# YukinoriMatsuoka/indy-plenum

Hardware: AMD Instinct MI355X
Metric: Ed25519 verifies/sec at 1/8 MI355X (256B msgs) + % of INT32 VALU peak vs host CPU (higher is better)
Workload: dtype int32

## Files before the change

indy-plenum_amd/csrc/edv_hostcheck.cpp:

```cpp
#include <stdint.h>
#include <string.h>
#include <vector>
#include "edv_verify_core.h"
#include "edv_sha256.h"
#include "edv_merkle.h"
#include "edv_ledger.h"
#include "edv_tables.h"
#include "edv_selftest_cases.h"
#include "edv_probe_ops.h"

using namespace edv;

namespace {
struct HostATab {
  ge_cached t[kAEntries];
  int staged = 0;
  void store(int e, const ge_cached& c) { t[e] = c; }
  ge_cached load(int e) const { return t[e]; }
  void stage(int e) { staged = e; }
  ge_cached fetch() const { return t[staged]; }
};
struct HostBTab {
  SbShape sh;
  ge_p3 base[kBTablesCompact];
  explicit HostBTab(SbShape s) : sh(s) {
    for (int t = 0; t < sh.tables; t++) base[t] = base_point(t * sh.bits);
  }
  ge_precomp entry(int t, int j) const {
    int32_t w[kBStride];
    btab_entry(w, j, base[t]);
    return precomp_from_words(w);
  }
};
struct HostBStage {
  const HostBTab& b;
  int t = 0, j = 0;
  ge_cached stash;
  SbShape shape() const { return b.sh; }
  void stage(int tt, int jj) { t = tt; j = jj; }
  ge_precomp fetch() const { return b.entry(t, j); }
  void put(const ge_cached& c) { stash = c; }
  ge_cached get() const { return stash; }
};
struct HostComb {
  std::vector<int32_t> w;
  HostComb() : w(kCombRows * kCombEntries * kBStride) {
    for (int i = 0; i < kCombRows; i++)
      for (int j = 0; j < kCombEntries; j++) comb_entry(w.data() + (i * kCombEntries + j) * kBStride, i, j);
  }
  ge_precomp entry(int i, int j) const { return precomp_from_words(w.data() + (i * kCombEntries + j) * kBStride); }
};
const HostComb& comb() {
  static HostComb c;
  return c;
}
static_assert(kBTablesCompact >= kBTables, "base[] holds the larger table count");
const HostBTab& btab(int bits = kBBits) {
  static HostBTab large(sb_large()), compact(sb_compact());
  return bits == kBBitsCompact ? compact : large;
}
void load_words(uint32_t* w, const uint8_t* b, int n) {
  for (int i = 0; i < n; i++) w[i] = uint32_t(b[4 * i]) | uint32_t(b[4 * i + 1]) << 8 | uint32_t(b[4 * i + 2]) << 16 | uint32_t(b[4 * i + 3]) << 24;
}
void store_words(uint8_t* b, const uint32_t* w, int n) {
  for (int i = 0; i < n; i++)
    for (int j = 0; j < 4; j++) b[4 * i + j] = uint8_t(w[i] >> (8 * j));
}
fe to_fe(const int32_t* l) { fe f; for (int i = 0; i < 10; i++) f.v[i] = l[i]; return f; }
void from_fe(int32_t* l, const fe& f) { for (int i = 0; i < 10; i++) l[i] = f.v[i]; }
}

extern "C" {
void hc_fe_mul(const int32_t* f, const int32_t* g, int32_t* h) { from_fe(h, fe_mul(to_fe(f), to_fe(g))); }
void hc_fe_sq(const int32_t* f, int32_t* h) { from_fe(h, fe_sq(to_fe(f))); }
void hc_fe_sq_floor(const int32_t* f, int32_t* h) { from_fe(h, fe_sq_floor(to_fe(f))); }
void hc_fe_sq2(const int32_t* f, int32_t* h) { from_fe(h, fe_sq2(to_fe(f))); }
void hc_fe_carry32(const int32_t* f, int32_t* h) { from_fe(h, fe_carry32(to_fe(f))); }
void hc_fe_invert(const int32_t* f, int32_t* h) { from_fe(h, fe_invert(to_fe(f))); }
void hc_fe_invert_safegcd(const int32_t* f, int32_t* h) { from_fe(h, fe_invert_safegcd(to_fe(f))); }
void hc_fe_pow22523(const int32_t* f, int32_t* h) { from_fe(h, fe_pow22523(to_fe(f))); }
void hc_fe_tobytes(const int32_t* f, uint8_t* out) { uint32_t w[8]; fe_tobytes(w, to_fe(f)); store_words(out, w, 8); }
void hc_fe_frombytes(const uint8_t* in, int32_t* h) { uint32_t w[8]; load_words(w, in, 8); from_fe(h, fe_frombytes(w)); }
void hc_sc_reduce(const uint8_t* in64, uint8_t* out32) {
  uint32_t w[16], o[8];
  load_words(w, in64, 16);
  sc_reduce(o, w);
  store_words(out32, o, 8);
}
void hc_hram(const uint8_t* R, const uint8_t* A, const uint8_t* m, uint64_t mlen, uint8_t* out64) {
  uint32_t r[8], a[8], o[16];
  load_words(r, R, 8);
  load_words(a, A, 8);
  std::vector<uint8_t> buf(mlen + 32, 0);
  if (mlen) memcpy(buf.data() + 16, m, mlen);
  hram(o, r, a, buf.data() + 16, mlen);
  store_words(out64, o, 16);
}
int hc_decompress_negate(const uint8_t* in, uint8_t* out) {
  uint32_t w[8], o[8];
  load_words(w, in, 8);
  ge_p3 p;
  const bool ok = ge_frombytes_negate(p, w);
  ge_p2_tobytes(o, ge_p3_to_p2(p));
  store_words(out, o, 8);
  return ok ? 0 : -1;
}
void hc_sha256(const uint8_t* m, uint64_t mlen, int misalign, uint8_t* out32) {
  std::vector<uint8_t> buf(mlen + 48, 0xA5);
  if (mlen) memcpy(buf.data() + 16 + misalign, m, mlen);
  uint32_t o[8];
  sha256_msg(o, buf.data() + 16 + misalign, mlen);
  store_words(out32, o, 8);
}
int hc_sha256_batch(const uint8_t* msgs, const uint64_t* off, uint64_t n, uint8_t* out, uint32_t) {
  for (uint64_t i = 0; i < n; i++) {
    const uint64_t mlen = off[i + 1] - off[i];
    std::vector<uint8_t> buf(mlen + 48, 0);
    if (mlen) memcpy(buf.data() + 16, msgs + off[i], mlen);
    uint32_t o[8];
    sha256_msg(o, buf.data() + 16, mlen);
    store_words(out + 32 * i, o, 8);
  }
  return 0;
}
int hc_btab_entries_of_bits(int bits, int t, const int32_t* js, int nj, int32_t* out) {
  if (bits != kBBits && bits != kBBitsCompact) return -1;
  const HostBTab& b = btab(bits);
  if (t < 0 || t >= b.sh.tables) return -1;
  for (int k = 0; k < nj; k++) {
    if (js[k] < 0 || js[k] >= b.sh.entries) return -1;
    btab_entry(out + size_t(k) * kBStride, js[k], b.base[t]);
  }
  return 0;
}
int hc_btab_entries_of(int t, const int32_t* js, int nj, int32_t* out) {
  return hc_btab_entries_of_bits(kBBits, t, js, nj, out);
}
int hc_rside_point_bits(int bits, const uint8_t* R32, const uint8_t* S32, uint8_t* out32) {
  struct Keep {
    ge_cached q;
    void store(int e, const ge_cached& c) { if (e == 1) q = c; }
  } tab;
  uint32_t R[8], S[8], o[8];
  load_words(R, R32, 8);
  load_words(S, S32, 8);
  if (bits != kBBits && bits != kBBitsCompact) return -1;
  HostBStage bs{btab(bits)};
  if (!prep_rpoint(R, S, tab, bs)) return -1;
  const fe two_y = fe_carry32(fe_add(tab.q.YpX, tab.q.YmX)), two_x = fe_carry32(fe_sub(tab.q.YpX, tab.q.YmX));
  ge_p2 p{two_x, two_y, fe_carry32(fe_add(tab.q.Z, tab.q.Z))};
  ge_p2_tobytes(o, p);
  store_words(out32, o, 8);
  return 0;
}
int hc_rside_point(const uint8_t* R32, const uint8_t* S32, uint8_t* out32) {
  return hc_rside_point_bits(kBBits, R32, S32, out32);
}
int hc_half_scalars(const uint8_t* h32, uint8_t* a32, uint8_t* u32) {
  uint32_t h[8], a[8], u[8];
  load_words(h, h32, 8);
  bool neg = false;
  half_scalars(h, a, u, neg);
  store_words(a32, a, 8);
  store_words(u32, u, 8);
  return neg ? 1 : 0;
}
int hc_probe_math(int op, const void* in, uint64_t in_stride, void* out, uint64_t out_stride, uint64_t n) {
  const ProbeSize sz = probe_size(op);
  if (!sz.in || probe_is_quad(op) || in_stride < sz.in || out_stride < sz.out || (in_stride & 3) || (out_stride & 3))
    return -1;
  for (uint64_t i = 0; i < n; i++) {
    const uint32_t* x = reinterpret_cast<const uint32_t*>(static_cast<const uint8_t*>(in) + i * in_stride);
    uint32_t* y = reinterpret_cast<uint32_t*>(static_cast<uint8_t*>(out) + i * out_stride);
    switch (op) {
#define HC_PROBE_CASE(OP) case OP: probe_lane_op<OP>(x, y); break;
      HC_PROBE_CASE(EDV_PROBE_FE_MUL)
      HC_PROBE_CASE(EDV_PROBE_FE_SQ)
      HC_PROBE_CASE(EDV_PROBE_FE_SQ2)
      HC_PROBE_CASE(EDV_PROBE_FE_SQ_FLOOR)
      HC_PROBE_CASE(EDV_PROBE_FE_TOBYTES)
      HC_PROBE_CASE(EDV_PROBE_FE_FROMBYTES)
      HC_PROBE_CASE(EDV_PROBE_FE_INVERT_SAFEGCD)
      HC_PROBE_CASE(EDV_PROBE_FE_POW22523)
      HC_PROBE_CASE(EDV_PROBE_SC_REDUCE)
      HC_PROBE_CASE(EDV_PROBE_HALF_SCALARS)
      HC_PROBE_CASE(EDV_PROBE_RECODE5)
      HC_PROBE_CASE(EDV_PROBE_APPROX_DIV)
      HC_PROBE_CASE(EDV_PROBE_FDIV_FLOOR)
      HC_PROBE_CASE(EDV_PROBE_EUCLID_DIV)
      HC_PROBE_CASE(EDV_PROBE_GE_FROMBYTES)
      HC_PROBE_CASE(EDV_PROBE_SC_MULADD)
      HC_PROBE_CASE(EDV_PROBE_RECODE8)
      HC_PROBE_CASE(EDV_PROBE_GE_P3_TOBYTES)
#undef HC_PROBE_CASE
      case EDV_PROBE_SCALARMULT_BASE: probe_scalarmult_base(x, y, comb()); break;
      default: return -1;
    }
  }
  return 0;
}
static_assert(kAEntries * 40 == 360, "a slot's table is 9 entries of 4 x 10 limbs");
int hc_stage_prep(const uint8_t* sigs, const uint8_t* pks, const uint8_t* msgs, const uint64_t* off, uint64_t n,
                  int bits, int side0, int nsides, int buckets, uint64_t cap, uint32_t* dig, uint8_t* alive,
                  int32_t* atab, int32_t* rtab, uint32_t* perm, uint8_t* accept) {
  if ((bits != kBBits && bits != kBBitsCompact) || n > cap || side0 < 0 || nsides < 1 || side0 + nsides > 3) return -1;
  const HostBTab& bt = btab(bits);
  if (buckets) {
    auto bucket = [&](uint64_t i) {
      const uint64_t nb = (64 + (off[i + 1] - off[i]) + 17 + 127) / 128;
      return nb < 63 ? nb : uint64_t(63);
    };
    uint64_t k = 0;
    bool one = true;
    for (uint64_t i = 1; i < n; i++) one = one && bucket(i) == bucket(0);
    for (uint64_t b = 0; b < 64 && !one; b++)
      for (uint64_t i = 0; i < n; i++)
        if (bucket(i) == b) perm[k++] = uint32_t(i);
    for (uint64_t i = 0; one && i < n; i++) perm[i] = uint32_t(i);
  }
  for (uint64_t j = 0; j < n; j++) {
    const uint64_t i = buckets ? perm[j] : j;
    uint32_t R[8], S[8], A[8];
    load_words(R, sigs + 64 * i, 8);
    load_words(S, sigs + 64 * i + 32, 8);
    load_words(A, pks + 32 * i, 8);
    for (int side = side0; side < side0 + nsides; side++) {
      bool ok;
      if (side == 0) {
        const uint64_t mlen = off[i + 1] - off[i];
        std::vector<uint8_t> buf(mlen + 32, 0);
        if (mlen) memcpy(buf.data() + 16, msgs + off[i], mlen);
        PrepDigits pd;
        ok = prep_one(R, S, A, buf.data() + 16, mlen, pd);
        if (ok) {
          for (int k = 0; k < 8; k++) {
            dig[uint64_t(k) * cap + j] = pd.da[k];
            dig[uint64_t(8 + k) * cap + j] = pd.db[k];
          }
          dig[16 * cap + j] = uint32_t(pd.nwin) | (pd.negR ? 0x100u : 0u);
        }
      } else {
        HostATab tab;
        if (side == 1) {
          ok = prep_point(A, tab);
        } else {
          HostBStage bs{bt};
          ok = prep_rpoint(R, S, tab, bs);
        }
        int32_t* o = (side == 1 ? atab : rtab) + j * 360;
        for (int e = 0; ok && e < kAEntries; e++) {
          from_fe(o + 40 * e, tab.t[e].YpX);
          from_fe(o + 40 * e + 10, tab.t[e].YmX);
          from_fe(o + 40 * e + 20, tab.t[e].Z);
          from_fe(o + 40 * e + 30, tab.t[e].T2d);
        }
      }
      alive[uint64_t(side) * cap + j] = ok ? 1 : 0;
      if (!ok) accept[i] = 0;
    }
  }
  return 0;
}
int hc_stage_main(uint64_t n, uint64_t cap, const uint32_t* dig, const uint8_t* alive, const int32_t* atab,
                  const int32_t* rtab, const uint32_t* perm, uint8_t* accept) {
  if (n > cap) return -1;
  auto live = [&](uint64_t j) { return j < n && alive[j] && alive[cap + j] && alive[2 * cap + j]; };
  for (uint64_t w0 = 0; w0 < n; w0 += 64) {
    int nwin = 0;
    for (uint64_t j = w0; j < w0 + 64; j++)
      if (live(j)) nwin = mx(nwin, int(dig[16 * cap + j] & 0xff));
    if (nwin > kAWindows) return -1;
    for (uint64_t j = w0; j < w0 + 64; j++) {
      if (!live(j)) continue;
      if (perm && perm[j] >= n) return -1;
      uint32_t da[8], db[8];
      for (int k = 0; k < 8; k++) {
        da[k] = dig[uint64_t(k) * cap + j];
        db[k] = dig[uint64_t(8 + k) * cap + j];
      }
      HostATab at, rt;
      for (int e = 0; e < kAEntries; e++) {
        const int32_t *a = atab + j * 360 + 40 * e, *r = rtab + j * 360 + 40 * e;
        at.t[e] = ge_cached{to_fe(a), to_fe(a + 10), to_fe(a + 20), to_fe(a + 30)};
        rt.t[e] = ge_cached{to_fe(r), to_fe(r + 10), to_fe(r + 20), to_fe(r + 30)};
      }
      accept[perm ? perm[j] : j] = main_one(da, db, nwin, (dig[16 * cap + j] >> 8) & 1, at, rt) ? 1 : 0;
    }
  }
  return 0;
}
namespace {
void put_p3(int32_t* pt, int k, uint64_t slots, uint64_t j, const ge_p3& p) {
  const fe* c[4] = {&p.X, &p.Y, &p.Z, &p.T};
  for (int q = 0; q < 4; q++)
    for (int i = 0; i < 10; i++) pt[(uint64_t(k) * 40 + 10 * q + i) * slots + j] = c[q]->v[i];
}
ge_p3 get_p3(const int32_t* pt, int k, uint64_t slots, uint64_t j) {
  fe c[4];
  for (int q = 0; q < 4; q++)
    for (int i = 0; i < 10; i++) c[q].v[i] = pt[(uint64_t(k) * 40 + 10 * q + i) * slots + j];
  return ge_p3{c[0], c[1], c[2], c[3]};
}
ge_p3 p3_add(const ge_p3& p, const ge_p3& q) { return ge_p1p1_to_p3(ge_add(p, ge_p3_to_cached(q))); }
ge_p3 p3_neg(const ge_p3& p) { return ge_p3{fe_neg(p.X), p.Y, p.Z, fe_neg(p.T)}; }
ge_p3 signed_digit_mult(const uint32_t d[8], bool negate, const ge_p3& P) {
  ge_p3 m[9];
  m[0] = ge_p3_identity();
  for (int e = 1; e < 9; e++) m[e] = p3_add(m[e - 1], P);
  ge_p3 acc = ge_p3_identity();
  for (int k = 63; k >= 0; k--) {
    for (int t = 0; t < 4; t++) acc = ge_p1p1_to_p3(ge_p2_dbl(ge_p3_to_p2(acc)));
    int dg = int(d[k / 8] >> (4 * (k % 8))) & 15;
    if (dg >= 8) dg -= 16;
    if (negate) dg = -dg;
    if (dg) acc = p3_add(acc, dg < 0 ? p3_neg(m[-dg]) : m[dg]);
  }
  return acc;
}
}
int hc_stage_latency_phase1(const uint8_t* sigs, const uint8_t* pks, const uint8_t* msgs, const uint64_t* off,
                            uint64_t n, int ns, int bits, uint32_t* dig, int32_t* pt, uint8_t* ok) {
  if ((bits != kBBits && bits != kBBitsCompact) || (ns != 16 && ns != 32) || n == 0) return -1;
  const HostBTab& bt = btab(bits);
  const uint64_t slots = (n + ns - 1) / ns * ns;
  for (uint64_t jl = 0; jl < slots; jl++) {
    const bool in = jl < n || jl < 16;
    const uint64_t i = jl < n ? jl : n - 1;
    bool ok0 = false, ok1 = false, ok2 = false;
    PrepDigits pd;
    ge_p3 pa = ge_p3_identity(), pr = ge_p3_identity(), sb = ge_p3_identity();
    if (in) {
      uint32_t R[8], S[8], A[8];
      load_words(R, sigs + 64 * i, 8);
      load_words(S, sigs + 64 * i + 32, 8);
      load_words(A, pks + 32 * i, 8);
      const uint64_t mlen = off[i + 1] - off[i];
      std::vector<uint8_t> buf(mlen + 32, 0);
      if (mlen) memcpy(buf.data() + 16, msgs + off[i], mlen);
      ok0 = prep_one(R, S, A, buf.data() + 16, mlen, pd);
      ok1 = ge_is_canonical(A) && !has_small_order(A) && ge_frombytes_negate(pa, A);
      if (!ok1) pa = ge_p3_identity();
      ok2 = ge_is_canonical(R) && !has_small_order(R) && ge_frombytes_negate(pr, R);
      if (!ok2) pr = ge_p3_identity();
      HostBStage bs{bt};
      add_sb(sb, S, bs);
    }
    for (int k = 0; k < 8; k++) {
      dig[uint64_t(k) * slots + jl] = ok0 ? pd.da[k] : 0u;
      dig[uint64_t(8 + k) * slots + jl] = ok0 ? pd.db[k] : 0u;
    }
    dig[16 * slots + jl] = ok0 ? (uint32_t(pd.nwin) | (pd.negR ? 0x100u : 0u)) : 0u;
    ok[jl] = ok0;
    ok[slots + jl] = ok1;
    ok[2 * slots + jl] = ok2;
    put_p3(pt, 0, slots, jl, pa);
    put_p3(pt, 1, slots, jl, pr);
    put_p3(pt, 2, slots, jl, sb);
  }
  return 0;
}
int hc_stage_latency_walk(uint64_t n, int ns, const uint32_t* dig, const int32_t* pt, const uint8_t* ok,
                          uint8_t* accept) {
  if ((ns != 16 && ns != 32) || n == 0) return -1;
  const uint64_t slots = (n + ns - 1) / ns * ns;
  for (uint64_t j = 0; j < n; j++) {
    const bool alive = ok[j] && ok[slots + j] && ok[2 * slots + j];
    if (!alive) {
      accept[j] = 0;
      continue;
    }
    const uint32_t wf = dig[16 * slots + j];
    if ((wf & 0xff) > uint32_t(kAWindows)) return -1;
    uint32_t da[8], db[8];
    for (int k = 0; k < 8; k++) {
      da[k] = dig[uint64_t(k) * slots + j];
      db[k] = dig[uint64_t(8 + k) * slots + j];
    }
    const ge_p3 q = p3_add(get_p3(pt, 2, slots, j), get_p3(pt, 1, slots, j));
    const ge_p3 r = p3_add(signed_digit_mult(da, false, get_p3(pt, 0, slots, j)),
                           signed_digit_mult(db, (wf >> 8) & 1, q));
    accept[j] = (fe_iszero(r.X) && fe_iszero(fe_sub(r.Y, r.Z))) ? 1 : 0;
  }
  return 0;
}
int hc_comb_entries(const int32_t* ij, int n, int32_t* out) {
  const HostComb& ct = comb();
// ... 185 lines not shown
```

indy-plenum_amd/csrc/edv_prep.hip:

```cpp
#define EDV_NO_SCHED_FENCE 1
#include <hip/hip_runtime.h>
#include <stdint.h>

#include "edv_kernels.h"

namespace edv {
namespace {



template <int BITS>
__device__ __forceinline__ void prep_point_side(const VerifyArgs& a, uint64_t j, int side, int32_t* lds) {
  if (j >= a.n) return;
  const uint64_t i = a.base + (a.st.perm ? a.st.perm[j] : j);
  uint32_t P[8];
  bool ok;
  if (side == 1) {
    load_words(P, a.pks + 8 * i, 2);
    GlobalATab tab{a.st.atab + j * kAWords};
    ok = prep_point(P, tab);
  } else {
    uint32_t S[8];
    load_words(P, a.sigs + 16 * i, 2);
    load_words(S, a.sigs + 16 * i + 8, 2);
    GlobalATab tab{a.st.rtab + j * kAWords};
    LdsBStage<BITS> bs{a.btab, lds + (threadIdx.x >> 6) * kLdsBWaveWords, int(threadIdx.x & 63)};
    ok = prep_rpoint(P, S, tab, bs);
  }
  a.st.alive[side * a.st.cap + j] = ok ? 1 : 0;
  if (!ok) a.accept[i] = 0;
}
template <int BITS>
__device__ __forceinline__ void prep_body(const VerifyArgs& a, int32_t* lds_b) {
  const uint32_t ns = uint32_t(a.nsides);
  const int side = a.side0 + int(blockIdx.x % ns);
  const uint64_t j = uint64_t(blockIdx.x / ns) * kBlock + threadIdx.x;
  if (side != 0) {
    prep_point_side<BITS>(a, j, side, lds_b);
    return;
  }
  if (j >= a.n) return;
  const uint64_t i = a.base + (a.st.perm ? a.st.perm[j] : j);
  uint32_t R[8], S[8], A[8];
  load_words(R, a.sigs + 16 * i, 2);
  load_words(S, a.sigs + 16 * i + 8, 2);
  load_words(A, a.pks + 8 * i, 2);
  const uint64_t o0 = a.off[i] - a.msg_base, o1 = a.off[i + 1] - a.msg_base;
  PrepDigits pd;
  const bool ok = prep_one(R, S, A, a.msgs + o0, o1 - o0, pd);
  a.st.alive[j] = ok ? 1 : 0;
  if (ok) {
    uint32_t* d = a.st.dig + j;
    const uint64_t cap = a.st.cap;
#pragma unroll
    for (int k = 0; k < 8; k++) {
      d[uint64_t(k) * cap] = pd.da[k];
      d[uint64_t(8 + k) * cap] = pd.db[k];
    }
    d[uint64_t(kDigNwin) * cap] = uint32_t(pd.nwin) | (pd.negR ? 0x100u : 0u);
  } else {
    a.accept[i] = 0;
  }
}

__global__ __launch_bounds__(kBlock) __attribute__((amdgpu_waves_per_eu(3, 8))) void edv_prep_kernel(
    VerifyArgs a) {
  extern __shared__ int32_t lds_b[];
  prep_body<kBBits>(a, lds_b);
}
__global__ __launch_bounds__(kBlock) __attribute__((amdgpu_waves_per_eu(3, 8))) void edv_prep_kernel_compact(
    VerifyArgs a) {
  extern __shared__ int32_t lds_b[];
  prep_body<kBBitsCompact>(a, lds_b);
}

}

hipError_t launch_prep_kernel(unsigned grid, hipStream_t s, const VerifyArgs& va) {
  const bool rside = va.side0 + va.nsides > 2;
  const size_t lds = rside ? size_t(kBlock / 64) * kLdsBWaveWords * sizeof(int32_t) : 0;
  if (va.sb.bits == kBBits) edv_prep_kernel<<<dim3(grid), dim3(kBlock), lds, s>>>(va);
  else edv_prep_kernel_compact<<<dim3(grid), dim3(kBlock), lds, s>>>(va);
  return hipGetLastError();
}

}
```

indy-plenum_amd/csrc/edv_verify_core.h:

```cpp
#pragma once
#include "edv_math.h"

namespace edv {

constexpr int kAWin = 4;
constexpr int kAWindows = (255 + kAWin - 1) / kAWin;
constexpr int kAEntries = (1 << (kAWin - 1)) + 1;
constexpr int kBBits = 22;
constexpr int kBTables = (253 + kBBits - 1) / kBBits;
constexpr int kBEntries = (1 << (kBBits - 1)) + 1;
constexpr int kBBitsCompact = 16;
constexpr int kBTablesCompact = (253 + kBBitsCompact - 1) / kBBitsCompact;
constexpr int kBEntriesCompact = (1 << (kBBitsCompact - 1)) + 1;
static_assert(253 - kBBits * (kBTables - 1) <= kBBits - 1, "top [S]B digit out of table range");
static_assert(253 - kBBitsCompact * (kBTablesCompact - 1) <= kBBitsCompact - 1, "top [S]B digit out of table range");
struct SbShape {
  int bits, tables, entries;
};
EDV_HD constexpr SbShape sb_large() { return SbShape{kBBits, kBTables, kBEntries}; }
EDV_HD constexpr SbShape sb_compact() { return SbShape{kBBitsCompact, kBTablesCompact, kBEntriesCompact}; }
constexpr int kCombEntries = 129;
constexpr int kBStride = 32;

EDV_HD int mx(int a, int b) { return a > b ? a : b; }
// ... 146 lines not shown
  for (int k = 0; k < kAWindows; k++) {
    const int pos = kAWin * k, wi = pos >> 5, sh = pos & 31;
    const uint64_t win = uint64_t(d[wi]) | (wi + 1 < 8 ? uint64_t(d[wi + 1]) << 32 : 0);
    n = ((win >> sh) & ((1u << kAWin) - 1)) ? k + 1 : n;
  }
  return n;
}

EDV_HD bool w8_lt(const uint32_t a[8], const uint32_t b[8]) {
  bool lt = false, eq = true;
#pragma unroll
  for (int i = 7; i >= 0; i--) {
    lt = lt || (eq && a[i] < b[i]);
    eq = eq && a[i] == b[i];
  }
  return lt;
}
EDV_HD void w8_add(uint32_t a[8], const uint32_t b[8]) {
  uint64_t c = 0;
#pragma unroll
  for (int i = 0; i < 8; i++) {
    c += uint64_t(a[i]) + b[i];
    a[i] = uint32_t(c);
    c >>= 32;
  }
}
EDV_HD void w8_sub(uint32_t a[8], const uint32_t b[8]) {
  int64_t br = 0;
#pragma unroll
  for (int i = 0; i < 8; i++) {
    const int64_t s = int64_t(a[i]) - int64_t(b[i]) + br;
    a[i] = uint32_t(s);
    br = s >> 32;
  }
}
EDV_HD double w8_to_f64(const uint32_t a[8]) {
  double d = 0.0;
#pragma unroll
  for (int i = 7; i >= 0; i--) d = d * 4294967296.0 + double(a[i]);
  return d;
}
EDV_HD void w8_shl1(uint32_t a[8]) {
#pragma unroll
  for (int i = 7; i > 0; i--) a[i] = (a[i] << 1) | (a[i - 1] >> 31);
  a[0] <<= 1;
}
EDV_HD void w8_sar1(uint32_t a[8]) {
#pragma unroll
  for (int i = 0; i < 7; i++) a[i] = (a[i] >> 1) | (a[i + 1] << 31);
  a[7] = uint32_t(int32_t(a[7]) >> 1);
}
EDV_HD void w8_shr1(uint32_t a[8]) {
#pragma unroll
  for (int i = 0; i < 7; i++) a[i] = (a[i] >> 1) | (a[i + 1] << 31);
  a[7] >>= 1;
}

#ifndef EDV_RCP_DIV
#define EDV_RCP_DIV 1
#endif
EDV_HD double approx_div(double a, double b) {
#if defined(__HIP_DEVICE_COMPILE__)
  if (EDV_RCP_DIV) {
    double r = __builtin_amdgcn_rcp(b);
    r = __builtin_fma(r, __builtin_fma(-b, r, 1.0), r);
    return a * r;
  }
#endif
  return a / b;
}
EDV_HD void euclid_div(uint32_t r0[8], uint32_t t0[8], const uint32_t r1[8], const uint32_t t1[8]) {
  const double qd = __builtin_floor(approx_div(w8_to_f64(r0), w8_to_f64(r1)) * (1.0 - 0x1p-44));
  uint32_t q = 0;
  if (qd < 2147483648.0) {
    q = uint32_t(qd);
    uint64_t c = 0;
    int64_t br = 0;
#pragma unroll
    for (int i = 0; i < 8; i++) {
      const uint64_t p = uint64_t(q) * r1[i] + c;
      c = p >> 32;
      const int64_t s = int64_t(r0[i]) - int64_t(uint32_t(p)) + br;
      r0[i] = uint32_t(s);
      br = s >> 32;
    }
  } else {
    uint32_t d[8], v[8];
#pragma unroll
    for (int i = 0; i < 8; i++) { d[i] = r1[i]; v[i] = t1[i]; }
    const int e = int((__builtin_bit_cast(uint64_t, qd * (1.0 + 0x1p-42)) >> 52) & 0x7ff) - 1023;
#pragma unroll 1
    for (int k = 0; k < e; k++) { w8_shl1(d); w8_shl1(v); }
#pragma unroll 1
    for (int k = e; k >= 0; k--) {
      if (!w8_lt(r0, d)) { w8_sub(r0, d); w8_sub(t0, v); }
      w8_shr1(d);
      w8_sar1(v);
    }
  }
  const uint32_t m = w8_lt(r0, r1) ? 0u : ~0u;
  int64_t br = 0;
#pragma unroll
  for (int i = 0; i < 8; i++) {
    const int64_t s = int64_t(r0[i]) - int64_t(r1[i] & m) + br;
    r0[i] = uint32_t(s);
    br = s >> 32;
  }
  q -= m;
  uint64_t c = 0;
  int64_t bt = 0;
#pragma unroll
  for (int i = 0; i < 8; i++) {
    const uint64_t p = uint64_t(q) * t1[i] + c;
    c = p >> 32;
    const int64_t s = int64_t(t0[i]) - int64_t(uint32_t(p)) + bt;
    t0[i] = uint32_t(s);
    bt = s >> 32;
  }
}

EDV_HD bool w8_ge128(const uint32_t r[8]) { return (r[4] | r[5] | r[6] | r[7]) != 0; }

EDV_HD double w8_window53(const uint32_t r[8], int s) {
  const int wi = s >> 5, b = s & 31;
  uint32_t w0 = 0, w1 = 0, w2 = 0;
#pragma unroll
  for (int k = 0; k < 8; k++) {
    const uint32_t d = uint32_t(k - wi);
    const uint32_t m0 = ~nz_mask(d), m1 = ~nz_mask(d - 1u), m2 = ~nz_mask(d - 2u);
    w0 |= r[k] & m0;
    w1 |= r[k] & m1;
    w2 |= r[k] & m2;
  }
  const uint64_t lo = (uint64_t(w1) << 32) | w0;
  const uint64_t v = b == 0 ? lo : ((lo >> b) | (uint64_t(w2) << (64 - b)));
  return double(v);
}
EDV_HD double fdiv_floor(double a, double b) {
  double q = __builtin_floor(approx_div(a, b));
  const double r = __builtin_fma(-q, b, a);
  q = r < 0 ? q - 1 : (r >= b ? q + 1 : q);
  return q;
}
EDV_HD void w8_lin(uint32_t out[8], const uint32_t x[8], const uint32_t y[8], int32_t a, int32_t b) {
  int64_t c = 0;
#pragma unroll
  for (int i = 0; i < 8; i++) {
    const int64_t v = int64_t(a) * int64_t(uint64_t(x[i])) + int64_t(b) * int64_t(uint64_t(y[i])) + c;
    out[i] = uint32_t(v);
    c = v >> 32;
  }
}

EDV_HD bool lehmer_round(uint32_t r0[8], uint32_t r1[8], uint32_t t0[8], uint32_t t1[8]) {
  const int n = w8_bitlen(r0);
  const int s = n > 53 ? n - 53 : 0;
  double x = w8_window53(r0, s), y = w8_window53(r1, s);
  const double thr = __builtin_ldexp(1.0, 128 - s);
  double A = 1, B = 0, C = 0, D = 1;
#pragma unroll 1
  for (int k = 0; k < 60; k++) {
    const double yc = y + C, yd = y + D;
    if (!(yc > 0 && yd > 0)) break;
    const double q = fdiv_floor(x + A, yc);
    const double r2 = __builtin_fma(-q, yd, x + B);
    if (!(r2 >= 0 && r2 < yd)) break;
    const double yn = x - q * y, Cn = A - q * C, Dn = B - q * D;
    if (yn - __builtin_fabs(Cn) - __builtin_fabs(Dn) < thr || __builtin_fabs(Cn) + __builtin_fabs(Dn) > 0x1p30) break;
    A = C; B = D; C = Cn; D = Dn;
    x = y; y = yn;
  }
  if (B == 0) return false;
  const int32_t a = int32_t(A), b = int32_t(B), c = int32_t(C), d = int32_t(D);
  uint32_t n0[8], n1[8];
  w8_lin(n0, r0, r1, a, b);
  w8_lin(n1, r0, r1, c, d);
#pragma unroll
  for (int i = 0; i < 8; i++) { r0[i] = n0[i]; r1[i] = n1[i]; }
  w8_lin(n0, t0, t1, a, b);
  w8_lin(n1, t0, t1, c, d);
#pragma unroll
  for (int i = 0; i < 8; i++) { t0[i] = n0[i]; t1[i] = n1[i]; }
  return true;
}

EDV_HD bool w8_neg_(const uint32_t t[8]) { return t[7] >> 31; }
EDV_HD void w8_abs(uint32_t out[8], const uint32_t t[8]) {
  const uint32_t m = w8_neg_(t) ? ~0u : 0u;
  uint64_t c = m & 1;
#pragma unroll
  for (int i = 0; i < 8; i++) {
    c += uint64_t(t[i] ^ m);
    out[i] = uint32_t(c);
    c >>= 32;
  }
}

EDV_HD void half_scalars(const uint32_t h[8], uint32_t a[8], uint32_t u[8], bool& neg) {
  uint32_t r0[8] = {0xe7ae9f68u, 0xc09318d2u, 0x17bce6b2u, 0xa6f7cef5u, 0u, 0u, 0u, 0x80000000u};
  uint32_t r1[8], t0[8], t1[8];
#pragma unroll
  for (int i = 0; i < 8; i++) { r1[i] = h[i]; t0[i] = 0; t1[i] = i == 0; }
#pragma unroll 1
  for (int it = 0; it < 40 && w8_bitlen(r1) > 140; it++) {
    if (!lehmer_round(r0, r1, t0, t1)) break;
  }
  bool flip = false;
  if (w8_ge128(r1)) {
#pragma unroll 1
    for (int it = 0; it < 200; it++) {
      euclid_div(r0, t0, r1, t1);
      if (!w8_ge128(r0)) { flip = true; break; }
      euclid_div(r1, t1, r0, t0);
      if (!w8_ge128(r1)) break;
    }
  }
  if (flip) {
#pragma unroll
    for (int i = 0; i < 8; i++) {
      const uint32_t tr = r0[i], tt = t0[i];
      r0[i] = r1[i]; t0[i] = t1[i];
      r1[i] = tr; t1[i] = tt;
    }
  }
  uint32_t u0[8], u1[8];
  w8_abs(u0, t0);
  w8_abs(u1, t1);
  const bool cur_ok = u1[0] & 1, prev_ok = u0[0] & 1;
  const int cur_len = mx(w8_bitlen(r1), w8_bitlen(u1)), prev_len = mx(w8_bitlen(r0), w8_bitlen(u0));
  if (cur_ok && (!prev_ok || cur_len <= prev_len)) {
#pragma unroll
    for (int i = 0; i < 8; i++) { a[i] = r1[i]; u[i] = u1[i]; }
    neg = w8_neg_(t1);
    return;
  }
#pragma unroll
  for (int i = 0; i < 8; i++) { a[i] = r0[i]; u[i] = u0[i]; }
  neg = w8_neg_(t0);
  if (!cur_ok && (r1[2] | r1[3])) {
    euclid_div(r0, t0, r1, t1);
    w8_abs(u0, t0);
    if (mx(w8_bitlen(r0), w8_bitlen(u0)) < prev_len) {
#pragma unroll
      for (int i = 0; i < 8; i++) { a[i] = r0[i]; u[i] = u0[i]; }
      neg = w8_neg_(t0);
    }
  }
}

template <int N>
EDV_HD void shl256(uint32_t v[8]) {
#pragma unroll
  for (int i = 7; i > 0; i--) v[i] = (v[i] << N) | (v[i - 1] >> (32 - N));
  v[0] <<= N;
}
template <int N>
EDV_HD void shr256(uint32_t v[8]) {
#pragma unroll
  for (int i = 0; i < 7; i++) v[i] = (v[i] >> N) | (v[i + 1] << (32 - N));
  v[7] >>= N;
}

EDV_HD ge_precomp precomp_from_words(const int32_t* w) {
  ge_precomp q;
#pragma unroll
  for (int l = 0; l < 10; l++) { q.ypx.v[l] = w[l]; q.ymx.v[l] = w[10 + l]; q.xy2d.v[l] = w[20 + l]; }
  return q;
}

EDV_HD ge_p3 base_point(int shift) {
  const uint32_t Bw[8] = {0x66666658u, 0x66666666u, 0x66666666u, 0x66666666u,
                          0x66666666u, 0x66666666u, 0x66666666u, 0x66666666u};
  ge_p3 nB;
  ge_frombytes_negate(nB, Bw);
  ge_p3 B{fe_neg(nB.X), nB.Y, nB.Z, fe_neg(nB.T)};
  for (int k = 0; k < shift; k++) B = ge_p1p1_to_p3(ge_p2_dbl(ge_p3_to_p2(B)));
  return B;
}
EDV_HD void btab_entry(int32_t* o, int j, const ge_p3& base) {
  const ge_cached Bc = ge_p3_to_cached(base);
  ge_p3 acc = ge_p3_identity();
  for (int bit = kBBits - 1; bit >= 0; bit--) {
    acc = ge_p1p1_to_p3(ge_p2_dbl(ge_p3_to_p2(acc)));
    if ((j >> bit) & 1) acc = ge_p1p1_to_p3(ge_add(acc, Bc));
  }
  const fe zi = fe_invert(acc.Z);
  const fe x = fe_mul(acc.X, zi), y = fe_mul(acc.Y, zi);
  const fe ypx = fe_carry32(fe_add(y, x)), ymx = fe_carry32(fe_sub(y, x));
  const fe xy2d = fe_mul(fe_mul(x, y), fe_d2());
  for (int l = 0; l < 10; l++) { o[l] = ypx.v[l]; o[10 + l] = ymx.v[l]; o[20 + l] = xy2d.v[l]; }
  o[30] = 0;
  o[31] = 0;
}

EDV_HD constexpr size_t sb_words(SbShape sh) { return size_t(sh.tables) * size_t(sh.entries) * kBStride; }
EDV_HD constexpr size_t sb_alloc_bytes(SbShape sh) { return 4 * sb_words(sh) + size_t(sh.tables) * sizeof(ge_p3); }

struct PrepDigits {
  uint32_t da[8];
  uint32_t db[8];
  int nwin;
  bool negR;
};

template <class Tab>
EDV_HD void build_table(Tab& tab, const ge_p3& P) {
  const ge_cached c1 = ge_p3_to_cached(P);
  const ge_precomp p1{c1.YpX, c1.YmX, c1.T2d};
  tab.store(0, ge_cached_identity());
  tab.store(1, c1);
  ge_p3 cur = ge_p1p1_to_p3(ge_p2_dbl(ge_p3_to_p2(P)));
  tab.store(2, ge_p3_to_cached(cur));
#pragma unroll 1
  for (int e = 3; e < kAEntries; e++) {
    cur = ge_p1p1_to_p3(ge_madd(cur, p1));
    tab.store(e, ge_p3_to_cached(cur));
  }
}
template <class Tab, class Stash>
EDV_HD void build_table_projective(Tab& tab, const ge_p3& P, Stash& st) {
  {
    const ge_cached c1 = ge_p3_to_cached(P);
    tab.store(0, ge_cached_identity());
    tab.store(1, c1);
    st.put(c1);
  }
  ge_p3 cur = ge_p1p1_to_p3(ge_p2_dbl(ge_p3_to_p2(P)));
  tab.store(2, ge_p3_to_cached(cur));
#pragma unroll 1
  for (int e = 3; e < kAEntries; e++) {
    cur = ge_p1p1_to_p3(ge_add(cur, st.get()));
    tab.store(e, ge_p3_to_cached(cur));
  }
}

EDV_HD bool prep_one(const uint32_t R[8], const uint32_t S[8], const uint32_t A[8], const uint8_t* m, uint64_t mlen,
                     PrepDigits& pd) {
  bool ok = !((S[7] & 0xF0000000u) && !sc_is_canonical(S));
  ok = ok && !has_small_order(R);
  ok = ok && ge_is_canonical(A) && !has_small_order(A);
  if (!ok) return false;
  uint32_t dig[16], h[8];
  hram(dig, R, A, m, mlen);
  sc_reduce(h, dig);
  uint32_t a[8], u[8];
  bool neg;
  half_scalars(h, a, u, neg);
  recode5(pd.da, a);
  recode5(pd.db, u);
  pd.nwin = mx(digits5_windows(pd.da), digits5_windows(pd.db));
  pd.negR = neg;
  return true;
}

template <class ATab>
EDV_HD bool prep_point(const uint32_t P[8], ATab& tab) {
  if (!ge_is_canonical(P) || has_small_order(P)) return false;
  ge_p3 nP;
  if (!ge_frombytes_negate(nP, P)) return false;
  build_table(tab, nP);
  return true;
}

EDV_HD void shr256_var(uint32_t v[8], int n) {
#pragma unroll
  for (int i = 0; i < 7; i++) v[i] = (v[i] >> n) | (v[i + 1] << (32 - n));
  v[7] >>= n;
}
template <class BTab>
EDV_HD void add_sb(ge_p3& q, const uint32_t S[8], BTab& bt) {
  const SbShape sh = bt.shape();
  uint32_t s[8];
#pragma unroll
  for (int i = 0; i < 8; i++) s[i] = S[i];
  s[7] &= 0x1fffffffu;
  int carry = 0;
  const int bits = sh.bits;
  auto next_digit = [&](bool top) {
    int e = int(s[0] & ((1u << bits) - 1)) + carry;
    shr256_var(s, bits);
    carry = top ? 0 : (e + (1 << (bits - 1))) >> bits;
    return e - carry * (1 << bits);
  };
  int dt = next_digit(sh.tables == 1);
  bt.stage(0, dt < 0 ? -dt : dt);
#pragma unroll 1
  for (int t = 0; t < sh.tables; t++) {
    const ge_precomp e = ge_precomp_cneg(bt.fetch(), dt < 0);
    if (t + 1 < sh.tables) {
      dt = next_digit(t + 2 == sh.tables);
      bt.stage(t + 1, dt < 0 ? -dt : dt);
    }
    q = ge_p1p1_to_p3(ge_madd(q, e));
  }
}
template <class BTab>
EDV_HD bool rpoint_q(const uint32_t R[8], const uint32_t S[8], BTab& bt, ge_p3& q) {
  if (!ge_is_canonical(R) || has_small_order(R)) return false;
  if (!ge_frombytes_negate(q, R)) return false;
  add_sb(q, S, bt);
  return true;
}
template <class ATab, class BTab>
EDV_HD bool prep_rpoint(const uint32_t R[8], const uint32_t S[8], ATab& tab, BTab& bt) {
  ge_p3 q;
  if (!rpoint_q(R, S, bt, q)) return false;
  build_table_projective(tab, q, bt);
  return true;
}

template <class ATab>
EDV_HD bool main_one(uint32_t da[8], uint32_t db[8], int nwin, bool negR, ATab& at, ATab& rt) {
  constexpr int kTop = kAWin * (kAWindows - 1);
  constexpr int kTopShl = 32 - kAWin - (kTop - 224);
#pragma unroll 1
  for (int k = nwin; k < kAWindows; k++) {
    shl256<kAWin>(da);
    shl256<kAWin>(db);
  }
  ge_p2 acc = ge_p2_identity();
#pragma unroll 1
  for (int w = nwin - 1; w >= 0; --w) {
    const int dA = int32_t(da[7] << kTopShl) >> (32 - kAWin);
    const int dR = int32_t(db[7] << kTopShl) >> (32 - kAWin);
    shl256<kAWin>(da);
    shl256<kAWin>(db);
    at.stage(dA < 0 ? -dA : dA);
    rt.stage(dR < 0 ? -dR : dR);
    ge_p3 p3;
    if (w == nwin - 1) {
      p3 = ge_p3_identity();
    } else {
#pragma unroll 1
      for (int d = 0; d < kAWin - 1; d++) acc = ge_p1p1_to_p2(ge_p2_dbl(acc));
      p3 = ge_p1p1_to_p3(ge_p2_dbl(acc));
    }
    const ge_cached ea = at.fetch();
    p3 = ge_p1p1_to_p3(ge_add(p3, ge_cached_cneg(ea, dA < 0)));
    const ge_cached er = rt.fetch();
    acc = ge_p1p1_to_p2(ge_add(p3, ge_cached_cneg(er, (dR < 0) != negR)));
  }
  return fe_iszero(acc.X) && fe_iszero(fe_carry32(fe_sub(acc.Y, acc.Z)));
}

template <class ATab, class BTab>
EDV_HD bool verify_one(const uint32_t R[8], const uint32_t S[8], const uint32_t A[8], const uint8_t* m, uint64_t mlen,
                       ATab& at, ATab& rt, BTab& bt) {
  PrepDigits pd;
  if (!prep_one(R, S, A, m, mlen, pd)) return false;
  if (!prep_point(A, at) || !prep_rpoint(R, S, rt, bt)) return false;
  return main_one(pd.da, pd.db, pd.nwin, pd.negR, at, rt);
}

constexpr int kCombRows = 32;
EDV_HD void comb_entry(int32_t* o, int i, int j) {
  const uint32_t Bw[8] = {0x66666658u, 0x66666666u, 0x66666666u, 0x66666666u,
                          0x66666666u, 0x66666666u, 0x66666666u, 0x66666666u};
  ge_p3 nB;
  ge_frombytes_negate(nB, Bw);
  ge_p3 base{fe_neg(nB.X), nB.Y, nB.Z, fe_neg(nB.T)};
  for (int k = 0; k < 8 * i; k++) base = ge_p1p1_to_p3(ge_p2_dbl(ge_p3_to_p2(base)));
  const ge_cached bc = ge_p3_to_cached(base);
  ge_p3 acc = ge_p3_identity();
  for (int bit = 7; bit >= 0; bit--) {
    acc = ge_p1p1_to_p3(ge_p2_dbl(ge_p3_to_p2(acc)));
    if ((j >> bit) & 1) acc = ge_p1p1_to_p3(ge_add(acc, bc));
  }
  const fe zi = fe_invert(acc.Z);
  const fe x = fe_mul(acc.X, zi), y = fe_mul(acc.Y, zi);
  const fe ypx = fe_carry32(fe_add(y, x)), ymx = fe_carry32(fe_sub(y, x));
  const fe xy2d = fe_mul(fe_mul(x, y), fe_d2());
  for (int l = 0; l < 10; l++) { o[l] = ypx.v[l]; o[10 + l] = ymx.v[l]; o[20 + l] = xy2d.v[l]; }
  o[30] = 0;
  o[31] = 0;
}
template <class CombTab>
EDV_HD ge_p3 scalarmult_base(const uint32_t k[8], const CombTab& ct) {
  uint32_t d[8];
  recode8(d, k);
  ge_p3 acc = ge_p3_identity();
#pragma unroll 1
  for (int i = 0; i < kCombRows; i++) {
    const int di = int(int8_t(uint8_t(d[i >> 2] >> (8 * (i & 3)))));
    const int ui = di < 0 ? -di : di;
    acc = ge_p1p1_to_p3(ge_madd(acc, ge_precomp_cneg(ct.entry(i, ui), di < 0)));
  }
  return acc;
}
EDV_HD void ge_p3_tobytes(uint32_t w[8], const ge_p3& p) { ge_p2_tobytes(w, ge_p3_to_p2(p)); }

EDV_HD void sc_muladd(uint32_t out[8], const uint32_t a[8], const uint32_t b[8], const uint32_t c[8]) {
  uint32_t t[16];
  uint64_t carry = 0;
#pragma unroll
  for (int k = 0; k < 16; k++) {
    uint64_t lo = carry + (k < 8 ? c[k] : 0), hi = 0;
#pragma unroll
    for (int i = 0; i < 8; i++) {
      const int j = k - i;
      if (j < 0 || j > 7) continue;
// ... 38 lines not shown
```

Before: 97.12 million.

## Speed up half-scalar lattice reduction with cheaper Lehmer steps and 5-word Euclid

Adds a batch variant of half_scalars used by the prep kernel and host check. The Lehmer inner loop gets an unrolled two-step form that swaps roles without copying and uses an approximate division checked by two remainders. The Euclid tail runs on 5-word (160-bit) operands with a single-word quotient and falls back to the 8-word path for large quotients. The aim is to cut integer and branch work in per-signature scalar preparation, at the cost of more code and correctness resting on the approximate-division bounds.

```diff
diff --git a/indy-plenum_amd/csrc/edv_hostcheck.cpp b/indy-plenum_amd/csrc/edv_hostcheck.cpp
--- a/indy-plenum_amd/csrc/edv_hostcheck.cpp
+++ b/indy-plenum_amd/csrc/edv_hostcheck.cpp
@@ -161,6 +161,15 @@
   load_words(h, h32, 8);
   bool neg = false;
   half_scalars(h, a, u, neg);
+  store_words(a32, a, 8);
+  store_words(u32, u, 8);
+  return neg ? 1 : 0;
+}
+int hc_half_scalars_batch(const uint8_t* h32, uint8_t* a32, uint8_t* u32) {
+  uint32_t h[8], a[8], u[8];
+  load_words(h, h32, 8);
+  bool neg = false;
+  half_scalars<true>(h, a, u, neg);
   store_words(a32, a, 8);
   store_words(u32, u, 8);
   return neg ? 1 : 0;
@@ -231,7 +240,7 @@
         std::vector<uint8_t> buf(mlen + 32, 0);
         if (mlen) memcpy(buf.data() + 16, msgs + off[i], mlen);
         PrepDigits pd;
-        ok = prep_one(R, S, A, buf.data() + 16, mlen, pd);
+        ok = prep_one<true>(R, S, A, buf.data() + 16, mlen, pd);
         if (ok) {
           for (int k = 0; k < 8; k++) {
             dig[uint64_t(k) * cap + j] = pd.da[k];
diff --git a/indy-plenum_amd/csrc/edv_prep.hip b/indy-plenum_amd/csrc/edv_prep.hip
--- a/indy-plenum_amd/csrc/edv_prep.hip
+++ b/indy-plenum_amd/csrc/edv_prep.hip
@@ -47,7 +47,7 @@
   load_words(A, a.pks + 8 * i, 2);
   const uint64_t o0 = a.off[i] - a.msg_base, o1 = a.off[i + 1] - a.msg_base;
   PrepDigits pd;
-  const bool ok = prep_one(R, S, A, a.msgs + o0, o1 - o0, pd);
+  const bool ok = prep_one<true>(R, S, A, a.msgs + o0, o1 - o0, pd);
   a.st.alive[j] = ok ? 1 : 0;
   if (ok) {
     uint32_t* d = a.st.dig + j;
diff --git a/indy-plenum_amd/csrc/edv_verify_core.h b/indy-plenum_amd/csrc/edv_verify_core.h
--- a/indy-plenum_amd/csrc/edv_verify_core.h
+++ b/indy-plenum_amd/csrc/edv_verify_core.h
@@ -322,6 +322,19 @@
   }
 }
 
+EDV_HD void lehmer_apply(uint32_t r0[8], uint32_t r1[8], uint32_t t0[8], uint32_t t1[8], int32_t a, int32_t b,
+                         int32_t c, int32_t d) {
+  uint32_t n0[8], n1[8];
+  w8_lin(n0, r0, r1, a, b);
+  w8_lin(n1, r0, r1, c, d);
+#pragma unroll
+  for (int i = 0; i < 8; i++) { r0[i] = n0[i]; r1[i] = n1[i]; }
+  w8_lin(n0, t0, t1, a, b);
+  w8_lin(n1, t0, t1, c, d);
+#pragma unroll
+  for (int i = 0; i < 8; i++) { t0[i] = n0[i]; t1[i] = n1[i]; }
+}
+
 EDV_HD bool lehmer_round(uint32_t r0[8], uint32_t r1[8], uint32_t t0[8], uint32_t t1[8]) {
   const int n = w8_bitlen(r0);
   const int s = n > 53 ? n - 53 : 0;
@@ -341,17 +354,111 @@
     x = y; y = yn;
   }
   if (B == 0) return false;
-  const int32_t a = int32_t(A), b = int32_t(B), c = int32_t(C), d = int32_t(D);
-  uint32_t n0[8], n1[8];
-  w8_lin(n0, r0, r1, a, b);
-  w8_lin(n1, r0, r1, c, d);
-#pragma unroll
-  for (int i = 0; i < 8; i++) { r0[i] = n0[i]; r1[i] = n1[i]; }
-  w8_lin(n0, t0, t1, a, b);
-  w8_lin(n1, t0, t1, c, d);
-#pragma unroll
-  for (int i = 0; i < 8; i++) { t0[i] = n0[i]; t1[i] = n1[i]; }
+  lehmer_apply(r0, r1, t0, t1, int32_t(A), int32_t(B), int32_t(C), int32_t(D));
   return true;
+}
+
+EDV_HD bool lehmer_step(double& A, double& B, double& x, double C, double D, double y, double thr) {
+  const double yc = y + C, yd = y + D;
+  if (!(yc > 0 && yd > 0)) return false;
+  const double xa = x + A;
+  const double q = __builtin_floor(approx_div(xa, yc));
+  const double e1 = __builtin_fma(-q, yc, xa), e2 = __builtin_fma(-q, yd, x + B);
+  if (!(e1 >= 0 && e1 < yc && e2 >= 0 && e2 < yd)) return false;
+  const double yn = x - q * y, Cn = A - q * C, Dn = B - q * D;
+  if (yn - __builtin_fabs(Cn) - __builtin_fabs(Dn) < thr || __builtin_fabs(Cn) + __builtin_fabs(Dn) > 0x1p30) return false;
+  A = Cn; B = Dn; x = yn;
+  return true;
+}
+EDV_HD bool lehmer_round_alt(uint32_t r0[8], uint32_t r1[8], uint32_t t0[8], uint32_t t1[8]) {
+  const int n = w8_bitlen(r0);
+  const int s = n > 53 ? n - 53 : 0;
+  double x = w8_window53(r0, s), y = w8_window53(r1, s);
+  const double thr = __builtin_ldexp(1.0, 128 - s);
+  double A = 1, B = 0, C = 0, D = 1;
+  bool odd = false;
+#pragma unroll 1
+  for (int k = 0; k < 30; k++) {
+    if (!lehmer_step(A, B, x, C, D, y, thr)) break;
+    odd = true;
+    if (!lehmer_step(C, D, y, A, B, x, thr)) break;
+    odd = false;
+  }
+  int32_t a = int32_t(A), b = int32_t(B), c = int32_t(C), d = int32_t(D);
+  const uint32_t m = odd ? ~0u : 0u;
+  const uint32_t sa = uint32_t(a ^ c) & m, sb = uint32_t(b ^ d) & m;
+  a ^= int32_t(sa); c ^= int32_t(sa);
+  b ^= int32_t(sb); d ^= int32_t(sb);
+  if (b == 0) return false;
+  lehmer_apply(r0, r1, t0, t1, a, b, c, d);
+  return true;
+}
+
+EDV_HD bool w5_lt(const uint32_t a[5], const uint32_t b[5]) {
+  bool lt = false, eq = true;
+#pragma unroll
+  for (int i = 4; i >= 0; i--) {
+    lt = lt || (eq && a[i] < b[i]);
+    eq = eq && a[i] == b[i];
+  }
+  return lt;
+}
+EDV_HD double w5_to_f64(const uint32_t a[5]) {
+  double d = 0.0;
+#pragma unroll
+  for (int i = 4; i >= 0; i--) d = d * 4294967296.0 + double(a[i]);
+  return d;
+}
+EDV_HD void w5_widen(uint32_t out[8], const uint32_t a[5], bool sign_extend) {
+  const uint32_t top = sign_extend ? uint32_t(int32_t(a[4]) >> 31) : 0u;
+#pragma unroll
+  for (int i = 0; i < 8; i++) out[i] = i < 5 ? a[i] : top;
+}
+EDV_HD void euclid_div5(uint32_t r0[5], uint32_t t0[5], const uint32_t r1[5], const uint32_t t1[5]) {
+  const double qd = __builtin_floor(approx_div(w5_to_f64(r0), w5_to_f64(r1)) * (1.0 - 0x1p-44));
+  if (!(qd < 2147483648.0)) {
+    uint32_t R0[8], T0[8], R1[8], T1[8];
+    w5_widen(R0, r0, false);
+    w5_widen(R1, r1, false);
+    w5_widen(T0, t0, true);
+    w5_widen(T1, t1, true);
+    euclid_div(R0, T0, R1, T1);
+#pragma unroll
+    for (int i = 0; i < 5; i++) { r0[i] = R0[i]; t0[i] = T0[i]; }
+    return;
+  }
+  uint32_t q = uint32_t(qd);
+  {
+    uint64_t c = 0;
+    int64_t br = 0;
+#pragma unroll
+    for (int i = 0; i < 5; i++) {
+      const uint64_t p = uint64_t(q) * r1[i] + c;
+      c = p >> 32;
+      const int64_t s = int64_t(r0[i]) - int64_t(uint32_t(p)) + br;
+      r0[i] = uint32_t(s);
+      br = s >> 32;
+    }
+  }
+  const uint32_t m = w5_lt(r0, r1) ? 0u : ~0u;
+  int64_t br = 0;
+#pragma unroll
+  for (int i = 0; i < 5; i++) {
+    const int64_t s = int64_t(r0[i]) - int64_t(r1[i] & m) + br;
+    r0[i] = uint32_t(s);
+    br = s >> 32;
+  }
+  q -= m;
+  uint64_t c = 0;
+  int64_t bt = 0;
+#pragma unroll
+  for (int i = 0; i < 5; i++) {
+    const uint64_t p = uint64_t(q) * t1[i] + c;
+    c = p >> 32;
+    const int64_t s = int64_t(t0[i]) - int64_t(uint32_t(p)) + bt;
+    t0[i] = uint32_t(s);
+    bt = s >> 32;
+  }
 }
 
 EDV_HD bool w8_neg_(const uint32_t t[8]) { return t[7] >> 31; }
@@ -366,6 +473,7 @@
   }
 }
 
+template <bool BATCH = false>
 EDV_HD void half_scalars(const uint32_t h[8], uint32_t a[8], uint32_t u[8], bool& neg) {
   uint32_t r0[8] = {0xe7ae9f68u, 0xc09318d2u, 0x17bce6b2u, 0xa6f7cef5u, 0u, 0u, 0u, 0x80000000u};
   uint32_t r1[8], t0[8], t1[8];
@@ -373,10 +481,25 @@
   for (int i = 0; i < 8; i++) { r1[i] = h[i]; t0[i] = 0; t1[i] = i == 0; }
 #pragma unroll 1
   for (int it = 0; it < 40 && w8_bitlen(r1) > 140; it++) {
-    if (!lehmer_round(r0, r1, t0, t1)) break;
+    if (!(BATCH ? lehmer_round_alt(r0, r1, t0, t1) : lehmer_round(r0, r1, t0, t1))) break;
   }
   bool flip = false;
-  if (w8_ge128(r1)) {
+  if (BATCH && w8_ge128(r1) && !(r0[5] | r0[6] | r0[7])) {
+    uint32_t p0[5], p1[5], c0[5], c1[5];
+#pragma unroll
+    for (int i = 0; i < 5; i++) { p0[i] = r0[i]; p1[i] = r1[i]; c0[i] = t0[i]; c1[i] = t1[i]; }
+#pragma unroll 1
+    for (int it = 0; it < 200; it++) {
+      euclid_div5(p0, c0, p1, c1);
+      if (!p0[4]) { flip = true; break; }
+      euclid_div5(p1, c1, p0, c0);
+      if (!p1[4]) break;
+    }
+    w5_widen(r0, p0, false);
+    w5_widen(r1, p1, false);
+    w5_widen(t0, c0, true);
+    w5_widen(t1, c1, true);
+  } else if (w8_ge128(r1)) {
 #pragma unroll 1
     for (int it = 0; it < 200; it++) {
       euclid_div(r0, t0, r1, t1);
@@ -504,6 +627,7 @@
   }
 }
 
+template <bool BATCH = false>
 EDV_HD bool prep_one(const uint32_t R[8], const uint32_t S[8], const uint32_t A[8], const uint8_t* m, uint64_t mlen,
                      PrepDigits& pd) {
   bool ok = !((S[7] & 0xF0000000u) && !sc_is_canonical(S));
@@ -515,7 +639,7 @@
   sc_reduce(h, dig);
   uint32_t a[8], u[8];
   bool neg;
-  half_scalars(h, a, u, neg);
+  half_scalars<BATCH>(h, a, u, neg);
   recode5(pd.da, a);
   recode5(pd.db, u);
   pd.nwin = mx(digits5_windows(pd.da), digits5_windows(pd.db));
```

Result: no change. 97.51 million, median of 6 (+0.4%).
